# xuelunshen/gim

Hardware: AMD Instinct MI355X
Metric: image-pairs/sec at 640x480 (higher is better)
Workload: dtype fp16

## Files before the change

gim_amd/_lib.py:

```python
import ctypes
import os

_HERE = os.path.dirname(os.path.abspath(__file__))
LIB_PATH = os.path.join(_HERE, "lib", "libgimhip.so")
if os.environ.get("GIM_LIB"):
    LIB_PATH = os.environ["GIM_LIB"] if os.path.isabs(os.environ["GIM_LIB"]) else os.path.join(os.path.dirname(_HERE), os.environ["GIM_LIB"])

GIM_F32, GIM_BF16, GIM_F16 = 0, 1, 2
ACT_NONE, ACT_RELU, ACT_LEAKY, ACT_ELU1, ACT_GELU = 0, 1, 2, 3, 4

c_void_p, c_int, c_int64, c_float = ctypes.c_void_p, ctypes.c_int, ctypes.c_int64, ctypes.c_float


class ConvArgs(ctypes.Structure):
    _fields_ = [
        ("x", c_void_p), ("w", c_void_p), ("ktab", c_void_p), ("bias", c_void_p), ("res", c_void_p),
        ("y", c_void_p), ("x_bytes", c_int64),
        ("B", c_int), ("H", c_int), ("W", c_int), ("Ho", c_int), ("Wo", c_int),
        ("stride", c_int), ("pad", c_int), ("ldx", c_int), ("ldy", c_int), ("ldres", c_int),
        ("N", c_int), ("npad", c_int), ("kpad", c_int), ("act", c_int), ("act_cols", c_int), ("res_mod", c_int),
        ("dtype", c_int), ("out_dtype", c_int), ("res_dtype", c_int), ("use_lds_dma", c_int),
        ("ups", c_void_p), ("ups_h", c_int), ("ups_w", c_int), ("ups_ld", c_int),
        ("health", c_void_p),
        ("split16", c_int), ("pad_", c_int),
# ... 106 lines not shown
    "gim_resize_bilinear": (c_int, [c_void_p] * 2 + [c_int] * 10 + [c_void_p]),
    "gim_resize_image": (c_int, [c_void_p] * 2 + [c_int] * 9 + [c_void_p]),
    "gim_grid_sample": (c_int, [c_void_p] * 3 + [c_int] * 9 + [c_void_p]),
    "gim_dkm_disp_emb": (c_int, [c_void_p] * 4 + [c_int] * 6 + [c_void_p]),
    "gim_local_corr": (c_int, [c_void_p] * 4 + [c_int] * 10 + [c_void_p]),
    "gim_dwconv5x5_bn_relu": (c_int, [c_void_p] * 5 + [c_int] * 9 + [c_void_p]),
    "gim_dwconv5x5_pw": (c_int, [c_void_p] * 7 + [c_int] * 7 + [c_void_p]),
    "gim_row_norms": (c_int, [c_void_p] * 2 + [c_int] * 4 + [c_void_p]),
    "gim_cos_kernel_finish": (c_int, [c_void_p] * 3 + [c_int] * 4 + [c_float] * 3 + [c_void_p]),
    "gim_gp_solve_ws_bytes": (c_int64, [c_int] * 3),
    "gim_gp_solve": (c_int, [c_void_p] * 4 + [c_int] * 5 + [c_void_p]),
    "gim_gp_posterior_f64_ws_bytes": (c_int64, [c_int] * 4),
    "gim_gp_posterior_f64": (c_int, [c_void_p] * 5 + [c_int] * 6 + [c_float] * 3 + [c_void_p]),
    "gim_global_avgpool": (c_int, [c_void_p] * 2 + [c_int] * 7 + [c_void_p]),
    "gim_cab_scale_add": (c_int, [c_void_p] * 4 + [c_int] * 8 + [c_void_p]),
    "gim_dkm_flow_update": (c_int, [c_void_p] * 3 + [c_int64, c_int, c_float, c_float, c_int, c_int, c_void_p]),
    "gim_dkm_grid_coords": (c_int, [c_void_p] + [c_int] * 3 + [c_void_p]),
    "gim_dkm_match_post": (c_int, [c_void_p] * 10 + [c_int] * 2 + [c_void_p]),
    "gim_dkm_black_mask": (c_int, [c_void_p] * 2 + [c_int] * 4 + [c_void_p]),
    "gim_kde": (c_int, [c_void_p] * 2 + [c_int, c_float, c_void_p]),
    "gim_cls_to_flow": (c_int, [c_void_p] * 3 + [c_int] * 3 + [c_void_p]),
    "gim_dense_to_pixels": (c_int, [c_void_p] * 3 + [c_int] + [c_float] * 4 + [c_void_p]),
    "gim_weighted_sample_ws_bytes": (c_int64, [c_int]),
    "gim_weighted_sample": (c_int, [c_void_p] * 3 + [c_int, c_int, ctypes.c_uint32, c_void_p]),
    "gim_ppm_pool": (c_int, [c_void_p] * 2 + [c_int] * 6 + [c_void_p]),
    "gim_ppm_upsample_concat": (c_int, [c_void_p] * 2 + [c_int] * 7 + [c_void_p]),
    "gim_seg_head_argmax": (c_int, [c_void_p] * 4 + [c_int] * 7 + [c_void_p]),
    "gim_slot_copy": (c_int, [c_void_p] * 4 + [c_int, c_int64, c_int, c_int, c_void_p]),
    "gim_nn_match_ws_bytes": (c_int64, [c_int] * 4),
    "gim_nn_match": (c_int, [c_void_p] * 2 + [c_int] * 4 + [c_float] + [c_void_p] * 5),
    "gim_conv3x3_halo_tiles": (c_int, [ctypes.POINTER(ConvArgs), c_void_p, c_void_p, c_int, c_void_p]),
    "gim_fine_tile_list_max_flags": (c_int, []),
    "gim_fine_tile_list": (c_int, [c_void_p] * 4 + [c_int] * 7 + [c_void_p, c_void_p, c_int, c_void_p]),
    "gim_ransac_score": (c_int, [c_void_p] * 5 + [c_int, c_int, ctypes.c_double, c_void_p, c_void_p]),
    "gim_ransac_mask": (c_int, [c_void_p] * 4 + [c_int, ctypes.c_double, c_void_p, c_void_p]),
}


class GimHipError(RuntimeError):
    pass


def _load():
    if not os.path.exists(LIB_PATH):
        raise ImportError(
            f"libgimhip.so not found at {LIB_PATH}: the HIP extension is required (no CPU fallback). "
            "Build it with `python -m gim_amd.build` (needs hipcc, gfx950).")
    try:
        import torch
    except ImportError:
        pass
    lib = ctypes.CDLL(LIB_PATH)
    for name, (res, args) in PROTOTYPES.items():
        fn = getattr(lib, name)
        fn.restype = res
        fn.argtypes = args
    if lib.gim_version() != ABI_VERSION:
        raise ImportError(f"{LIB_PATH} is ABI revision {lib.gim_version()}, gim_amd/_lib.py binds revision {ABI_VERSION}: rebuild with `python -m gim_amd.build`")
    return lib


lib = _load()


def check(rc, what=""):
    if rc != 0:
# ... 3 lines not shown
```

gim_amd/csrc/emit.hip:

```cpp
#include "gim_common.h"

namespace {

struct Segs { gim_copy_segs s; };

__global__ void __launch_bounds__(256) copy_segments_kernel(const Segs a) {
    const int k = blockIdx.y;
    const char* src = (const char*)a.s.src[k];
    char* dst = (char*)a.s.dst[k];
    const int64_t n = a.s.bytes[k];
    const int64_t t = (int64_t)blockIdx.x * blockDim.x + threadIdx.x, nt = (int64_t)gridDim.x * blockDim.x;
    const bool vec = (((uintptr_t)src | (uintptr_t)dst) & 15) == 0;
    const int64_t nv = vec ? n >> 4 : 0;
    for (int64_t i = t; i < nv; i += nt) ((uint4*)dst)[i] = src ? ((const uint4*)src)[i] : make_uint4(0u, 0u, 0u, 0u);
    for (int64_t i = (nv << 4) + t; i < n; i += nt) dst[i] = src ? src[i] : (char)0;
}

__global__ void __launch_bounds__(256) pack_matches_kernel(const int64_t* __restrict__ m_bids, const float2* __restrict__ mk0,
                                                           const float2* __restrict__ mk1, const float* __restrict__ conf,
                                                           const int64_t* __restrict__ pair_ids, int64_t pid_base,
                                                           float* __restrict__ out, int M) {
    const int m = blockIdx.x * blockDim.x + threadIdx.x;
    if (m >= M) return;
    const int64_t b = m_bids[m];
    const float pid = (float)(pair_ids ? pair_ids[b] : pid_base + b);
    const float2 p0 = mk0[m], p1 = mk1[m];
    float* o = out + (size_t)m * 6;
    *(float2*)(o + 0) = make_float2(pid, p0.x);
    *(float2*)(o + 2) = make_float2(p0.y, p1.x);
    *(float2*)(o + 4) = make_float2(p1.y, conf[m]);
}

constexpr int TL_THREADS = 1024, TL_MAX_FLAGS = 32768;

__global__ void __launch_bounds__(TL_THREADS) fine_tile_list_kernel(const int64_t* __restrict__ b_ids, const int64_t* __restrict__ i_ids,
                                                                  const int64_t* __restrict__ j_ids, const int* __restrict__ count, int cap,
                                                                  int bs, int w0c, int w1c, int stride, int H, int W,
                                                                  int* __restrict__ tiles, int* __restrict__ n_tiles, int tiles_cap) {
    __shared__ unsigned char flags[TL_MAX_FLAGS];
    __shared__ int part[TL_THREADS];
    const int t = threadIdx.x;
    const int tiles_x = (W + 31) / 32, tiles_y = (H + 7) / 8, per_img = tiles_x * tiles_y, nflags = 2 * bs * per_img;
    for (int i = t; i < nflags; i += TL_THREADS) flags[i] = 0;
    __syncthreads();
    int M = count[0];
    M = M < 0 ? 0 : (M < cap ? M : cap);
    for (int m = t; m < M; m += TL_THREADS) {
        const int64_t b = b_ids[m];
        if (b < 0 || b >= bs) continue;
#pragma unroll
        for (int side = 0; side < 2; ++side) {
            const int64_t cell = side ? j_ids[m] : i_ids[m];
            const int wc = side ? w1c : w0c;
            if (cell < 0 || cell >= (int64_t)wc * ((H + stride - 1) / stride)) continue;
            const int cy = (int)cell / wc, cx = (int)cell - cy * wc;
            int y0 = cy * stride - 3, y1 = cy * stride + 3, x0 = cx * stride - 3, x1 = cx * stride + 3;
            y0 = y0 < 0 ? 0 : y0; x0 = x0 < 0 ? 0 : x0;
            y1 = y1 > H - 1 ? H - 1 : y1; x1 = x1 > W - 1 ? W - 1 : x1;
            if (y0 > y1 || x0 > x1) continue;
            const int img = side * bs + (int)b;
            for (int ty = y0 >> 3; ty <= (y1 >> 3); ++ty)
                for (int tx = x0 >> 5; tx <= (x1 >> 5); ++tx) flags[(img * tiles_y + ty) * tiles_x + tx] = 1;
        }
    }
    __syncthreads();
    const int per = (nflags + TL_THREADS - 1) / TL_THREADS;
    const int lo = t * per < nflags ? t * per : nflags, hi = lo + per < nflags ? lo + per : nflags;
    int n = 0;
    for (int i = lo; i < hi; ++i) n += flags[i];
    part[t] = n;
    __syncthreads();
    for (int d = 1; d < TL_THREADS; d <<= 1) {
        const int v = t >= d ? part[t - d] : 0;
        __syncthreads();
        part[t] += v;
        __syncthreads();
    }
    int o = part[t] - n;
    for (int i = lo; i < hi; ++i)
        if (flags[i]) {
            if (o < tiles_cap) tiles[o] = i;
            ++o;
        }
    if (t == TL_THREADS - 1) n_tiles[0] = part[t] < tiles_cap ? part[t] : tiles_cap;
}

}

extern "C" int gim_fine_tile_list_max_flags(void) { return TL_MAX_FLAGS; }

extern "C" int gim_fine_tile_list(const int64_t* b_ids, const int64_t* i_ids, const int64_t* j_ids, const int* count, int cap, int bs,
                                  int w0c, int w1c, int stride, int H, int W, int* tiles, int* n_tiles, int tiles_cap, gim_stream_t stream) {
    GIM_REQUIRE(b_ids && i_ids && j_ids && count && tiles && n_tiles, "gim_fine_tile_list: NULL pointer");
    GIM_REQUIRE(cap >= 0 && bs > 0 && w0c > 0 && w1c > 0 && stride > 0 && H > 0 && W > 0, "gim_fine_tile_list: bad geometry");
    const int64_t nflags = 2ll * bs * ((W + 31) / 32) * ((H + 7) / 8);
    GIM_REQUIRE(nflags <= TL_MAX_FLAGS, "gim_fine_tile_list: %lld patches exceed the %d flags of the one-workgroup kernel", (long long)nflags, TL_MAX_FLAGS);
    GIM_REQUIRE(tiles_cap >= nflags, "gim_fine_tile_list: the list holds %d entries, the maps have %lld patches", tiles_cap, (long long)nflags);
    hipLaunchKernelGGL(fine_tile_list_kernel, dim3(1), dim3(TL_THREADS), 0, (hipStream_t)stream, b_ids, i_ids, j_ids, count, cap, bs, w0c, w1c,
                       stride, H, W, tiles, n_tiles, tiles_cap);
    return gim_check_launch("fine_tile_list_kernel");
}

extern "C" int gim_copy_segments(const gim_copy_segs* sp, gim_stream_t stream) {
    GIM_REQUIRE(sp, "gim_copy_segments: NULL args");
    GIM_REQUIRE(sp->n >= 0 && sp->n <= GIM_MAX_COPY_SEGS, "gim_copy_segments: n=%d outside [0, %d]", sp->n, GIM_MAX_COPY_SEGS);
    int64_t mx = 0;
    for (int k = 0; k < sp->n; ++k) {
        GIM_REQUIRE(sp->bytes[k] >= 0 && (sp->bytes[k] == 0 || sp->dst[k]), "gim_copy_segments: segment %d: bad size / NULL dst", k);
        mx = sp->bytes[k] > mx ? sp->bytes[k] : mx;
    }
    if (sp->n == 0 || mx == 0) return GIM_OK;
    Segs a;
    a.s = *sp;
    int64_t blocks = (mx / 16 + 255) / 256;
    blocks = blocks < 1 ? 1 : (blocks > 1024 ? 1024 : blocks);
    hipLaunchKernelGGL(copy_segments_kernel, dim3((unsigned)blocks, (unsigned)sp->n), dim3(256), 0, (hipStream_t)stream, a);
    return gim_check_launch("copy_segments_kernel");
}

extern "C" int gim_pack_matches(const int64_t* m_bids, const float* mkpts0, const float* mkpts1, const float* mconf,
                                const int64_t* pair_ids, int64_t pid_base, float* out, int M, gim_stream_t stream) {
    GIM_REQUIRE(M >= 0, "gim_pack_matches: M=%d", M);
    if (M == 0) return GIM_OK;
    GIM_REQUIRE(m_bids && mkpts0 && mkpts1 && mconf && out, "gim_pack_matches: NULL pointer");
    hipLaunchKernelGGL(pack_matches_kernel, dim3((unsigned)((M + 255) / 256)), dim3(256), 0, (hipStream_t)stream, m_bids,
                       (const float2*)mkpts0, (const float2*)mkpts1, mconf, pair_ids, pid_base, out, M);
    return gim_check_launch("pack_matches_kernel");
}
```

gim_amd/loftr/loftr.py:

```python
import collections
import contextlib
import math
import os
import warnings

import torch
import torch.nn as nn

from .. import ops
from ..switches import flag
from .._lib import ACT_ELU1, ACT_LEAKY, ACT_NONE, ACT_RELU, GIM_F16, GimHipError
from ..packing import (PRECISION_DTYPE as _DT, PackedStem, cstore, is_half, pack_bneck, pack_bneck_ds, pack_bneck_tail, pack_conv, pack_conv_split, pack_fine_fused,
                       pack_stem7x7, pack_token_mlp, pack_token_emit, split_channels, torch_dtype)

SPLIT16_WSCALE, SPLIT16_LIMIT = 4096.0, 65504.0


def _half(v):
    return (v - 1) // 2 + 1


def split16_weight_overflow(packs):
    named = [(k, v.w) for k, v in packs.items() if hasattr(v, "w") and torch.is_tensor(v.w) and v.w.dtype == torch.float32 and v.w.numel()]
    if not named:
# ... 140 lines not shown
        if config["fine_concat_coarse_feat"]:
            raise NotImplementedError("fine_concat_coarse_feat=True is not used by gim_loftr and is not built")
        self.precision = _precision_from(config)
        self.coarse_sim = self._check_sim((config.get("coarse_sim") or flag("coarse_sim", "") or self.precision).lower())
        self.stem_fp16 = flag("stem_fp16", True, config)
        self.stem_split = flag("stem_split", "auto", config)
        self.stem_kernel = flag("stem_kernel", True, config)
        self.fp16_overflowed = False
        self.split_overflowed = False
        self.backbone = _ResNetFPN_8_2(config["resnetfpn"])
        self.loftr_coarse = _LocalFeatureTransformer(config["coarse"])
        self.loftr_fine = _LocalFeatureTransformer(config["fine"])
        self.W = config["fine_window_size"]
        self.use_lds_dma = flag("lds_dma", True, config)
        self.fine_fused = flag("fine_fused", True, config)
        self.token_fused = flag("token_fused", True, config)
        self.fine_dev_count = flag("fine_dev_count", True, config)
        self._count_pin = None
        self.token_emit = flag("token_emit", True, config)
        self.bneck_fused = flag("bneck_fused", True, config)
        self.bneck_tail = flag("bneck_tail", True, config)
        self.bneck_ds = flag("bneck_ds", True, config)
        self.bneck_tail_ds = flag("bneck_tail_ds", True, config)
        self.depth_groups = flag("depth_groups", 1, config)
        self.l3_chains = flag("l3_chains", 2, config)
        self.fp32_split = flag("fp32_split", True, config)
        self.trunk_chains = flag("trunk_chains", False, config)
        self.tf_chains = flag("tf_chains", 2, config)
        self.kv_fused = flag("kv_fused", True, config)
        self.q_local = flag("q_local", True, config)
        self.kv_init = flag("kv_init", True, config)
        self.pos_fused = flag("pos_fused", True, config)
        self.fine_sparse = flag("fine_sparse", True, config)
        self._packed = None
        self._health = None
        self._health_sync_left = 3
        self._split16 = None
        self._packed_key = None
        self._pe_cache = {}
        self.debug = None
        self.use_graph = flag("graph", True, config)
        self.graph_cache_size = max(1, flag("graph_cache", 4, config))
        self._graphs = collections.OrderedDict()
        self._seen = collections.OrderedDict()
        self._generation = 0
        self._weights_gen = getattr(self, "_weights_gen", 0)
        if config.get("weight") is not None:
            self.load_state_dict(torch.load(config["weight"], map_location="cpu"))

    def load_state_dict(self, state_dict, *args, **kwargs):
        for k in list(state_dict.keys()):
            if k.startswith("model."):
                state_dict[k.replace("model.", "", 1)] = state_dict.pop(k)
            if k.startswith("matcher."):
                state_dict[k.replace("matcher.", "", 1)] = state_dict.pop(k)
        self._invalidate()
        return super().load_state_dict(state_dict, *args, **kwargs)

    def _invalidate(self):
        self._packed = None
        self._health_sync_left = 3
        self._weights_gen = getattr(self, "_weights_gen", 0) + 1
        if hasattr(self, "_graphs"):
            self._graphs.clear()
            self._seen.clear()

# ... 153 lines not shown
            self._pe_cache[key] = pe.permute(1, 2, 0).reshape(h * w, d_model).contiguous().to(device)
        return self._pe_cache[key]

    @contextlib.contextmanager
    def _launch_scope(self, device):
        if self.precision == "fp32" and self.fp32_split and device is not None:
            self._prepack(device)
        outer = self._split16
        self._split16 = True if (self.precision == "fp32" and self.fp32_split) else None
        try:
            yield
        finally:
            self._split16 = outer

    def _conv(self, x, pk, act=ACT_NONE, **kw):
        return ops.conv2d(x, pk, act, lds_dma=self.use_lds_dma, health=self._health, split16=self._split16, **kw)

    def _linear(self, x, pk, y, act=ACT_NONE, **kw):
        ops.linear(x, pk, y, act, self.use_lds_dma, health=self._health, split16=self._split16, **kw)

    def _to_nhwc(self, images, dt, out=None):
        H, W = images[0].shape[2:]
        B = sum(im.shape[0] for im in images)
        split = self._split()
        if out is None:
            cs = 8 if self._stem_k() else cstore(split_channels(images[0].shape[1]) if split else 3, dt)
            out = torch.empty(B, H, W, cs, dtype=torch_dtype(dt), device=images[0].device)
        off = 0
        for im in images:
            (ops.nchw_to_nhwc_split if split else ops.nchw_to_nhwc)(im, out, off)
            off += im.shape[0]
        return out

    def _backbone(self, P, x, dt, fine_tail=True):
        x1, x2, x3_out = self._backbone_trunk(P, x, dt)
        x1_out = self._fpn_fine(P, x1, x2, x3_out)
        return x3_out, (self._fpn_fine_tail(P, x1_out) if fine_tail else x1_out)

    def _backbone_trunk(self, P, x, dt):
        B = x.shape[0]
        K = self.l3_chains if (self.debug is None and self.l3_chains > 1 and B % self.l3_chains == 0) else 1
        if K > 1:
            h4, w4 = _half(_half(x.shape[1])), _half(_half(x.shape[2]))
            if (B // K * h4 * w4) % 256 != 0 or (B // K * _half(h4) * _half(w4)) % 256 != 0:
                K = 1
        whole = K > 1 and self.trunk_chains
        G = K if whole else (self.depth_groups if (self.debug is None and self.depth_groups > 1 and B % self.depth_groups == 0) else 1)
        o3 = None
        if G > 1:
            n = B // G
            H1, W1 = _half(x.shape[1]), _half(x.shape[2])
            H2, W2 = _half(H1), _half(W1)
            tdt = torch_dtype(dt)
            x1 = torch.empty(B, H1, W1, P["l1.2.c3"].n_store, dtype=tdt, device=x.device)
            x2 = torch.empty(B, H2, W2, P["l2.3.c3"].n_store, dtype=tdt, device=x.device)
            if self.bneck_tail and "l2.3.tail" in P and (n * H2 * W2) % 256 == 0 and n * H2 * W2 * 1024 < (1 << 32) - 16:
                o3 = torch.empty(B, H2, W2, P["l3.0.c1"].n_store, dtype=tdt, device=x.device)

        def trunk12_group(g):
            sl = slice(g * n, (g + 1) * n)
            a1, a2, ao = self._trunk12(P, x[sl], dt, out=(x1[sl], x2[sl], o3[sl] if o3 is not None else None))
            assert (ao is None) == (o3 is None)
            for dst, src in ((x1, a1), (x2, a2), (o3, ao)):
                if src is not None and src.data_ptr() != dst[sl].data_ptr():
                    ops.copy_segments([(src.contiguous(), dst[sl])])

        if G == 1:
            x1, x2, o3 = self._trunk12(P, x, dt)
# ... 53 lines not shown
            p = f"l{li}.{bi}."
            last = bi == nblk - 1
            outs = out_last if last else None
            if o is None:
                o = self._conv(x, P[p + "c1"], ACT_RELU)
            if fuse and self.bneck_ds and (p + "fused_ds") in P and x.shape[3] == 64 and x.is_contiguous():
                x, o = ops.bneck64_ds(o, x, P[p + "fused_ds"], out=outs, health=self._health)
                continue
            rows_ds = x.shape[0] * _half(x.shape[1]) * _half(x.shape[2])
            if (self.bneck_tail and self.bneck_tail_ds and (p + "tail_ds") in P and x.is_contiguous() and x.shape[3] == 256
                    and rows_ds % 256 == 0 and rows_ds * 512 * 2 < (1 << 32) - 16):
                o = self._conv(o, P[p + "c2"], ACT_RELU)
                x, o = ops.bneck_tail_ds(o, x, P[p + "tail_ds"], out=outs, health=self._health)
                continue
            idn = self._conv(x, P[p + "ds"], ACT_NONE) if (p + "ds") in P else x
            if fuse:
                x, o = ops.bneck64(o, idn, P[p + "fused"], True, out=outs, health=self._health)
                continue
            o = self._conv(o, P[p + "c2"], ACT_RELU)
            rows = o.shape[0] * o.shape[1] * o.shape[2]
            if self.bneck_tail and (p + "tail") in P and rows % 256 == 0 and rows * 4 * o.shape[3] * 2 < (1 << 32) - 16:
                if li == 3 and last:
                    x, x3_out = ops.bneck_tail(o, idn.contiguous(), P[p + "tail"], ACT_NONE, store_x=self.debug is not None, out=outs,
                                               health=self._health)
                    o = None
                else:
                    x, o = ops.bneck_tail(o, idn.contiguous(), P[p + "tail"], out=outs, health=self._health)
                continue
            x = self._conv(o, P[p + "c3"], ACT_RELU, res=idn)
            o = None
        return x, o, x3_out

    def _fpn_fine(self, P, x1, x2, x3_out):
        x2_out = self._conv(x2, P["l2o"], ups=x3_out)
        x2_out = self._conv(self._conv(x2_out, P["l2o2a"], ACT_LEAKY), P["l2o2b"])
        return self._conv(x1, P["l1o"], ups=x2_out)

    def _fine_halo(self, P, h2, w2):
        return bool(self.fine_sparse and is_half(self._dt()) and self.use_lds_dma and ops.HALO and P["l1o2a"].halo is not None
                    and P["l1o2b"].halo is not None and h2 % 8 == 0 and w2 % 32 == 0)

    def _fpn_fine_tail(self, P, x1_out, tiles=None, n_tiles=None):
        B, H, W, _ = x1_out.shape
        if self._fine_halo(P, H, W):
            mid = torch.empty(B, H, W, P["l1o2a"].n_store, dtype=x1_out.dtype, device=x1_out.device)
            f = torch.empty(B, H, W, P["l1o2b"].n_store, dtype=x1_out.dtype, device=x1_out.device)
            ops.conv3x3_halo(x1_out, P["l1o2a"], mid, ACT_LEAKY, tiles=tiles, n_tiles=n_tiles)
            ops.conv3x3_halo(mid, P["l1o2b"], f, ACT_NONE, tiles=tiles, n_tiles=n_tiles)
            return f
        assert tiles is None
        return self._conv(self._conv(x1_out, P["l1o2a"], ACT_LEAKY), P["l1o2b"])

    def _fine_sparse_ok(self, P, xs):
        if self.debug is not None or len(xs) != 1:
            return False
        B, H, W = xs[0].shape[:3]
        h2, w2 = _half(H), _half(W)
        h8, w8 = _half(_half(h2)), _half(_half(w2))
        return self._fine_halo(P, h2, w2) and h2 == 4 * h8 and w2 == 4 * w8 and B * (h2 // 8) * (w2 // 32) <= ops.FINE_TILE_MAX_FLAGS

    def _fine_tail_sparse(self, P, x1_out, cr, bs):
        _, H, W, _ = x1_out.shape
        tiles, n_tiles = ops.fine_tile_list(cr.b_ids, cr.i_ids, cr.j_ids, cr.count, bs, cr.args.w0c, cr.args.w1c, 4, H, W)
        return self._fpn_fine_tail(P, x1_out, tiles, n_tiles)

    class _TfBuffers:
        _LAZY = {"QKV": 3, "QKV2": 3, "MSG": 1, "MRG": 1, "HID": 2, "MLP": 1}

        def __init__(self, R, C, tdt, dev):
            f32 = torch.float32
            self._shape = (R, C, tdt, dev)
            self.X32 = torch.empty(R, C, dtype=f32, device=dev)
            self.CAT = torch.empty(R, 2 * C, dtype=tdt, device=dev)
            self.ws = None
            self.MASK = None
            self.pos = None
            self.pos_all = None

        def __getattr__(self, name):
            w = type(self)._LAZY.get(name)
            if w is None:
                raise AttributeError(name)
            R, C, tdt, dev = self._shape
            t = torch.empty(R, w * C, dtype=tdt, device=dev)
            setattr(self, name, t)
            return t

    def _encoder_layer(self, P, p, T, xs, ss, nb, L, S, H, have_q=False, with_q_of_source=False):
        C = T.X32.shape[1]
        x_t, s_t = T.CAT[xs, :C], T.CAT[ss, :C]
        if xs == ss:
            self._linear(x_t, P[p + "qkv"], T.QKV[xs], ACT_ELU1, act_cols=2 * C)
        else:
            if not have_q:
                self._linear(x_t, P[p + "q_proj"], T.QKV[xs, :C], ACT_ELU1)
            if with_q_of_source:
                self._linear(s_t, P[p + "qkv"], T.QKV[ss], ACT_ELU1, act_cols=2 * C)
# ... 212 lines not shown
            if T.pos[sd] is not None:
                feat, pe = T.pos[sd]
                ops.posenc_add(feat, pe, T.X32[rows[sd]], T.CAT[rows[sd], :C])
                T.pos[sd] = None

    def _transformer(self, P, name, tf, T, n0, L, n1, S):
        r0, r1 = slice(0, n0 * L), slice(n0 * L, n0 * L + n1 * S)
        rall = slice(0, n0 * L + n1 * S)
        H = tf.nhead
        if (self.token_emit and self.token_fused and (name + ".emit", L == S) in P and L % 64 == 0 and S % 64 == 0 and H == 8
                and T.X32.shape[1] == 256 and all(f"{name}{li}.tok" in P for li in range(len(tf.layer_names)))):
            return self._transformer_emit(P, name, tf, T, n0, L, n1, S)
        self._posenc(T, (r0, r1))
        for li, kind in enumerate(tf.layer_names):
            p = f"{name}{li}."
            if kind == "self":
                if L == S:
                    self._encoder_layer(P, p, T, rall, rall, n0 + n1, L, S, H)
                else:
                    self._encoder_layer(P, p, T, r0, r0, n0, L, L, H)
                    self._encoder_layer(P, p, T, r1, r1, n1, S, S, H)
            else:
                self._encoder_layer(P, p, T, r0, r1, n0, L, S, H, with_q_of_source=True)
                self._encoder_layer(P, p, T, r1, r0, n1, S, L, H, have_q=True)

    def _coarse_stage(self, xs, bs, scale0, scale1, mask0=None, mask1=None, count=None):
        dev = xs[0].device
        if count is None:
            count = torch.zeros(2 + bs, dtype=torch.int32, device=dev)
        self._health = self._health_word(count[1:2])
        P = self._prepack(dev)
        if len(xs) == 1:
            if self._fine_sparse_ok(P, xs):
                c_all, x1_out = self._extract_stage(P, xs[0], fine_tail=False)
                st = self._match_stage(P, c_all[:bs], c_all[bs:], None, None, c_all, bs, xs[0].shape[1], scale0, scale1, mask0, mask1, count)
                f_all = self._fine_tail_sparse(P, x1_out, st["cr"], bs)
                st["f0"], st["f1"] = f_all[:bs], f_all[bs:]
                return st
            c_all, f_all = self._extract_stage(P, xs[0])
            c0, c1 = c_all[:bs], c_all[bs:]
            f0, f1 = f_all[:bs], f_all[bs:]
        else:
            c_all = None
            c0, f0 = self._extract_stage(P, xs[0])
            c1, f1 = self._extract_stage(P, xs[1])
        return self._match_stage(P, c0, c1, f0, f1, c_all, bs, xs[0].shape[1], scale0, scale1, mask0, mask1, count)

    def _health_word(self, word):
        split = ops.FP32_SPLIT if self._split16 is None else self._split16
        return word if (self.precision == "fp16" or (self.precision == "fp32" and split)) else None

    def _extract_stage(self, P, x, fine_tail=True):
        return self._backbone(P, x, self._dt(), fine_tail)

    def _match_stage(self, P, c0, c1, f0, f1, c_all, bs, H0, scale0, scale1, mask0, mask1, count):
        dev = c0.device
        dt = self._dt()
        self._health = self._health_word(count[1:2])
        tdt = torch_dtype(dt)
        cfg = self.config
        hw0_c, hw1_c = c0.shape[1:3], c1.shape[1:3]
        C = cfg["coarse"]["d_model"]
        L, S = hw0_c[0] * hw0_c[1], hw1_c[0] * hw1_c[1]
        T = self._TfBuffers(bs * (L + S), C, tdt, dev)
        r0, r1 = slice(0, bs * L), slice(bs * L, bs * (L + S))
        if mask0 is not None:
            T.MASK = torch.empty(bs * (L + S), dtype=torch.uint8, device=dev)
            T.MASK[r0].copy_(mask0.reshape(-1))
            T.MASK[r1].copy_(mask1.reshape(-1))
        T.pos = [(c0.reshape(-1, C), self._pos_encoding(C, *hw0_c, dev)), (c1.reshape(-1, C), self._pos_encoding(C, *hw1_c, dev))]
        T.pos_all = c_all.reshape(-1, C) if c_all is not None else None
        self._transformer(P, "c", self.loftr_coarse, T, bs, L, bs, S)
        mc = cfg["match_coarse"]
        scale = H0 / hw0_c[0]
        if is_half(dt) and self.coarse_sim == self.precision:
            fc0 = T.CAT[r0].view(bs, L, 2 * C)[:, :, :C]
            fc1 = T.CAT[r1].view(bs, S, 2 * C)[:, :, :C]
        else:
            fc0, fc1 = T.X32[r0].view(bs, L, C), T.X32[r1].view(bs, S, C)
        cr = ops.coarse_match(fc0, fc1, hw0_c, hw1_c, scale,
                              mc["dsmax_temperature"], mc["thr"], mc["border_rm"], scale0, scale1,
                              T.MASK[r0] if mask0 is not None else None, T.MASK[r1] if mask0 is not None else None, count=count)
        self._health = None
        return {"c0": c0, "c1": c1, "f0": f0, "f1": f1, "cr": cr,
                "feat_c0": T.X32[r0].view(bs, L, C), "feat_c1": T.X32[r1].view(bs, S, C)}

    def _graph_key(self, color0, color1, scale0, mask0):
        return (tuple(color0.shape), tuple(color1.shape), scale0 is not None, mask0 is not None, self.precision, bool(self.fp32_split),
                bool(self.fine_sparse), self.coarse_sim, self._img_dt(), self._split(), self._stem_k(), str(color0.device))

    def _stage_graphed(self, key, fill, warm, stage, bs, dev, scale0, scale1, mask0, mask1):
        ent = self._graphs.get(key)
        if ent is None:
            warm()
            sin = [fill(None),
                   scale0.clone().float() if scale0 is not None else None,
                   scale1.clone().float() if scale1 is not None else None,
                   mask0.clone() if mask0 is not None else None, mask1.clone() if mask1 is not None else None,
                   torch.zeros(2 + bs, dtype=torch.int32, device=dev)]
            torch.cuda.synchronize()
            graph = torch.cuda.CUDAGraph()
            with torch.cuda.graph(graph, capture_error_mode="thread_local"):
                out = stage(*sin)
            while len(self._graphs) >= self.graph_cache_size:
                self._graphs.popitem(last=False)
            ent = self._graphs[key] = (graph, sin, out)
        else:
            self._graphs.move_to_end(key)
            fill(ent[1][0])
        graph, sin, out = ent
        small = []
        if scale0 is not None:
            small += [(scale0, sin[1]), (scale1, sin[2])]
        if mask0 is not None:
            small += [(mask0, sin[3]), (mask1, sin[4])]
        ops.copy_segments(small)
        graph.replay()
        return out

    def _run_stage(self, key, graphed, eager):
        counted = self.use_graph and self.debug is None
        if counted and (key in self._graphs or self._seen.get(key, 0) >= 1):
# ... 30 lines not shown

    @torch.no_grad()
    def forward(self, data):
        c0 = data.get("color0")
        with self._launch_scope(c0.device if torch.is_tensor(c0) and c0.is_cuda else None):
            return self._forward(data)

    def _forward(self, data):
        for k in ("image0", "image1", "color0", "color1"):
            if k not in data:
                raise KeyError(f"LoFTR.forward needs data[{k!r}] (loftr.py:54-63)")
        color0, color1 = data["color0"], data["color1"]
        if not color0.is_cuda:
            raise GimHipError("gim_amd LoFTR runs on the HIP device only (no CPU fallback): move the inputs "
                              "and the module to 'cuda'")
        dev = color0.device
        self._prepack(dev)
        color0 = color0.contiguous().float()
        color1 = color1.contiguous().float()
        scale0, scale1, mask0, mask1 = self._pair_inputs(data, dev, (color0.shape[0], color0.shape[2] // 8, color0.shape[3] // 8),
                                                         (color1.shape[0], color1.shape[2] // 8, color1.shape[3] // 8))
        data.update({"bs": data["image0"].size(0),
                     "hw0_i": data["image0"].shape[2:], "hw1_i": data["image1"].shape[2:]})
        bs = data["bs"]
        groups = [[color0, color1]] if color0.shape[2:] == color1.shape[2:] else [[color0], [color1]]

        def to_nhwc(out):
            if out is None:
                return [self._to_nhwc(g, self._img_dt()) for g in groups]
            for g, x in zip(groups, out):
                self._to_nhwc(g, self._img_dt(), out=x)

        def warm():
            self._prepack(dev)
            for c in (color0, color1):
                self._pos_encoding(self.config["coarse"]["d_model"], _half(_half(_half(c.shape[2]))), _half(_half(_half(c.shape[3]))), dev)

        key = self._graph_key(color0, color1, scale0, mask0)
        st, graphed = self._run_stage(
            key, lambda: self._stage_graphed(key, to_nhwc, warm, lambda xs, *rest: self._coarse_stage(xs, color0.shape[0], *rest), color0.shape[0], dev,
                                             scale0, scale1, mask0, mask1),
            lambda: self._coarse_stage(to_nhwc(None), bs, scale0, scale1, mask0, mask1))
        return self._finish(data, st, graphed, scale1, lambda: self.forward(data))

    def _finish(self, data, st, graphed, scale1, rerun):
        dev = st["c0"].device
        c0, c1, f0, f1, cr = st["c0"], st["c1"], st["f0"], st["f1"], st["cr"]
        if self.debug is not None:
            self.debug.update({k: st[k] for k in ("c0", "c1", "f0", "f1", "feat_c0", "feat_c1")})
        hw0_c, hw1_c = c0.shape[1:3], c1.shape[1:3]
        hw0_f, hw1_f = f0.shape[1:3], f1.shape[1:3]
        data.update({"hw0_c": torch.Size(hw0_c), "hw1_c": torch.Size(hw1_c),
                     "hw0_f": torch.Size(hw0_f), "hw1_f": torch.Size(hw1_f)})

        fine = None
        dev_count = (self.fine_dev_count and self.fine_fused and self.debug is None and "fine_fused" in self._prepack(dev)
                     and f0.dtype in ops.HALF)
        if self._count_pin is None:
            self._count_pin = torch.empty(2, dtype=torch.int32).pin_memory()
        if dev_count:
            self._count_pin.copy_(cr.count[:2], non_blocking=True)
            ev = torch.cuda.Event()
            ev.record()
            cap = cr.b_ids.numel()
            fine = self._fine_level(f0, f1, cr.b_ids, cr.i_ids, cr.j_ids, cr.mkpts1_c, scale1, "scale0" in data,
                                    hw0_c, hw1_c, data["hw0_i"], True, count=cr.count)
            ev.synchronize()
# ... 202 lines not shown
```

gim_amd/ops.py:

```python
import ctypes
import os

import torch

from . import _lib
from ._lib import ACT_ELU1, ACT_GELU, ACT_LEAKY, ACT_NONE, ACT_RELU, GIM_BF16, GIM_F16, GIM_F32, check, lib
from .packing import elem_size, torch_dtype
from .switches import flag

_DT = {torch.float32: GIM_F32, torch.bfloat16: GIM_BF16, torch.float16: GIM_F16}
HALF = (torch.bfloat16, torch.float16)


PROFILE = None
PROFILE_FUSED = None


def _stream():
    return ctypes.c_void_p(torch.cuda.current_stream().cuda_stream)


class _Timed:

    def __init__(self, family, flops):
# ... 261 lines not shown
        launch = lambda: check(lib.gim_conv3x3_halo_tiles(ctypes.byref(a), _p(tiles), _p(n_tiles), tiles.numel(), _stream()),
                               "gim_conv3x3_halo_tiles")
    if PROFILE is None:
        launch()
        return
    e0, e1 = torch.cuda.Event(enable_timing=True), torch.cuda.Event(enable_timing=True)
    e0.record()
    launch()
    e1.record()
    label = f"{pk.cin}->{pk.cout} k3s1 M={B * H * W} halo"
    if tiles is None:
        PROFILE.append((e0, e1, 2.0 * B * H * W * pk.cout * pk.cin * 9, label))
    else:
        PROFILE.append((e0, e1, 2.0 * int(n_tiles[0].item()) * 256 * pk.cout * pk.cin * 9, label + " sparse"))


FINE_TILE_MAX_FLAGS = lib.gim_fine_tile_list_max_flags()


def fine_tile_list(b_ids, i_ids, j_ids, count, bs, w0c, w1c, stride, H, W, tiles=None, n_tiles=None):
    _req_cuda(b_ids, i_ids, j_ids, count, tiles, n_tiles)
    assert b_ids.dtype == i_ids.dtype == j_ids.dtype == torch.int64 and count.dtype == torch.int32
    assert b_ids.is_contiguous() and i_ids.is_contiguous() and j_ids.is_contiguous()
    cap = min(b_ids.numel(), i_ids.numel(), j_ids.numel())
    total = 2 * bs * ((H + 7) // 8) * ((W + 31) // 32)
    if tiles is None:
        tiles = torch.empty(total, dtype=torch.int32, device=b_ids.device)
    if n_tiles is None:
        n_tiles = torch.empty(1, dtype=torch.int32, device=b_ids.device)
    assert tiles.dtype == n_tiles.dtype == torch.int32 and tiles.is_contiguous()
    check(lib.gim_fine_tile_list(_p(b_ids), _p(i_ids), _p(j_ids), _p(count), cap, bs, w0c, w1c, stride, H, W, _p(tiles), _p(n_tiles),
                                 tiles.numel(), _stream()), "gim_fine_tile_list")
    return tiles, n_tiles


def linear(x, pk, y, act=ACT_NONE, lds_dma=True, act_cols=0, health=None, split16=None):
    rows = x.shape[0]
    conv_rows(x, pk, (1, 1, rows, 1, rows), y, act, None, 0, lds_dma, act_cols, health=health, split16=split16)


def upsample2x_add(x, y):
    _req_cuda(x, y)
    B, h, w, C = x.shape
    assert y.shape == (B, 2 * h, 2 * w, C) and x.dtype == y.dtype
    check(lib.gim_upsample2x_add(_p(x), _p(y), B, h, w, C, C, C, gim_dtype(x), _stream()), "gim_upsample2x_add")


def posenc_add(x, pe, out_f32, out_t):
    _req_cuda(x, pe, out_f32, out_t)
    R, C = x.shape
    check(lib.gim_posenc_add(_p(x), _p(pe), _p(out_f32), _p(out_t), R, pe.shape[0], C, x.stride(0),
                             out_f32.stride(0) if out_f32 is not None else 4,
                             out_t.stride(0) if out_t is not None else 4, gim_dtype(x), _stream()), "gim_posenc_add")


def layernorm_residual(x, gamma, beta, res, out_f32, out_t, eps=1e-5):
    _req_cuda(x, gamma, beta, res, out_f32, out_t)
    R, C = x.shape
    dt = gim_dtype(out_t) if out_t is not None else GIM_F32
    check(lib.gim_layernorm_residual(_p(x), _p(gamma), _p(beta), _p(res), _p(out_f32), _p(out_t), R, C,
                                     x.stride(0), res.stride(0) if res is not None else 4,
                                     out_f32.stride(0) if out_f32 is not None else 4,
                                     out_t.stride(0) if out_t is not None else 4, gim_dtype(x), dt, eps, _stream()),
          "gim_layernorm_residual")


# ... 789 lines not shown
```

include/gim_hip.h:

```cpp
#ifndef GIM_HIP_H
#define GIM_HIP_H
#include <stdint.h>

#ifdef __cplusplus
extern "C" {
#endif

typedef void* gim_stream_t;

enum { GIM_F32 = 0, GIM_BF16 = 1, GIM_F16 = 2 };
enum { GIM_ACT_NONE = 0, GIM_ACT_RELU = 1, GIM_ACT_LEAKY = 2, GIM_ACT_ELU1 = 3 , GIM_ACT_GELU = 4  };
enum { GIM_OK = 0, GIM_ERR_INVALID = -1, GIM_ERR_LAUNCH = -2, GIM_ERR_UNSUPPORTED = -3 };

int gim_version(void);
const char* gim_last_error(void);
int gim_ktile_bytes(void);
int gim_npad_granule(void);

int gim_nchw_to_nhwc(const float* src, void* dst, int B, int C, int H, int W, int cpad, int ld,
                     int b_off, int dtype, gim_stream_t stream);
int gim_nchw_to_nhwc_split(const float* src, void* dst, int B, int C, int H, int W, int ld, int b_off, int dtype,
                           gim_stream_t stream);

int64_t gim_stem7x7_weight_bytes(int split);
// ... 224 lines not shown
    const float* match_b;
    void* ws;
    int64_t* matches0;
    int64_t* matches1;
    float* mscores0;
    float* mscores1;
    int32_t* pos;
    int32_t* count;
    int B, M, N, C;
    int ld_desc;
    float threshold;
} gim_lg_assign_args;
int64_t gim_lg_assign_ws_bytes(int B, int M, int N, int C);
int gim_lg_assign(const gim_lg_assign_args* a, gim_stream_t stream);
int gim_lg_log_assignment(const gim_lg_assign_args* a, float* out, gim_stream_t stream);
int gim_lg_emit_matches(const int64_t* matches0, const float* mscores0, const int32_t* pos,
                        const int32_t* count, const float* kpts0, const float* kpts1, const float* scale0,
                        const float* scale1, int64_t* matches, float* scores, float* mkpts0, float* mkpts1,
                        int64_t* m_bids, int B, int M, int N, gim_stream_t stream);

enum { GIM_MAX_COPY_SEGS = 12 };
typedef struct gim_copy_segs {
    const void* src[12];
    void* dst[12];
    int64_t bytes[12];
    int n;
} gim_copy_segs;
int gim_copy_segments(const gim_copy_segs* segs, gim_stream_t stream);
int gim_pack_matches(const int64_t* m_bids, const float* mkpts0, const float* mkpts1, const float* mconf,
                     const int64_t* pair_ids, int64_t pid_base, float* out, int M, gim_stream_t stream);
int gim_fine_tile_list_max_flags(void);
int gim_fine_tile_list(const int64_t* b_ids, const int64_t* i_ids, const int64_t* j_ids, const int* count, int cap, int bs,
                       int w0c, int w1c, int stride, int H, int W, int* tiles, int* n_tiles, int tiles_cap, gim_stream_t stream);


int gim_maxpool3x3s2(const void* x, void* y, int B, int H, int W, int C, int ldx, int ldy, int dtype,
                     gim_stream_t stream);
int gim_resize_bilinear(const void* x, void* y, int B, int h, int w, int Ho, int Wo, int C, int ldx, int ldy,
                        int dtype, int out_dtype, gim_stream_t stream);
int gim_resize_image(const float* x, void* y, int B, int C, int h, int w, int Ho, int Wo, int cpad, int b_off,
                     int out_dtype, gim_stream_t stream);
int gim_grid_sample(const void* feat, const float* grid_xy, void* out, int B, int h, int w, int Ho, int Wo, int C,
                    int ldf, int ldo, int dtype, gim_stream_t stream);
int gim_dkm_disp_emb(const float* flow, const float* wgt, const float* bias, void* out, int B, int h, int w, int E,
                     int ldo, int out_dtype, gim_stream_t stream);
int gim_local_corr(const void* f0, const void* f1, const float* flow, void* out, int B, int h, int w, int C, int r,
                   int ld0, int ld1, int ldo, int dtype, int out_dtype, gim_stream_t stream);
int gim_dwconv5x5_bn_relu(const void* x, const float* wgt, const float* scale, const float* shift, void* y, int B,
                          int H, int W, int Cin, int Cout, int cpad, int ldx, int ldy, int dtype, gim_stream_t stream);
int gim_dwconv5x5_pw(const void* x, const float* wgt, const float* scale, const float* shift, const void* pw_w, const float* pw_b, void* y,
                     int B, int H, int W, int cs, int ldx, int ldy, int dtype, gim_stream_t stream);
int gim_row_norms(const void* x, float* out, int rows, int C, int ld, int dtype, gim_stream_t stream);
int gim_cos_kernel_finish(float* k, const float* nx, const float* ny, int B, int n, int m, int ld, float T, float eps,
                          float diag_add, gim_stream_t stream);
int64_t gim_gp_solve_ws_bytes(int B, int n, int nrhs);
int gim_gp_solve(const float* K, const float* F, float* Xt, void* ws, int B, int n, int ldk, int nrhs, int npad,
                 gim_stream_t stream);
int64_t gim_gp_posterior_f64_ws_bytes(int B, int n, int d, int nrhs);
int gim_gp_posterior_f64(const float* X, const float* Y, const float* F, float* mu, void* ws, int B, int n, int d, int ldx,
                         int nrhs, int ld_mu, float T, float eps, float sigma, gim_stream_t stream);
int gim_global_avgpool(const void* x, float* out, int B, int HW, int C, int ld, int ldo, int c_off, int dtype,
                       gim_stream_t stream);
int gim_cab_scale_add(const float* g, const void* x1, const void* x2, void* out, int B, int HW, int C, int ldg, int ld1,
                      int ld2, int ldo, int dtype, gim_stream_t stream);
int gim_dkm_flow_update(float* flow, float* cert, const void* d, int64_t npix, int ldd, float sx, float sy,
                        int cert_init, int dtype, gim_stream_t stream);
// ... 38 lines not shown
```

Baseline: 917.8.

## Compute FPN quarter-resolution tail only on tiles feeding matched fine windows

Extends the sparse fine-stage approach to the 1/4-resolution FPN refinement convs (l2o2a/l2o2b). After coarse matching, a single kernel builds two tile lists, one for 1/2 resolution and one for the dilated 1/4-resolution footprint, and the quarter-res 3x3 convs run through the halo-tile path over only those tiles. The goal is to skip convolution work in regions no fine window reads. In exchange, the backbone is split around coarse matching, persistent zeroed buffers are kept per shape and per graph, and the kernel adds more bookkeeping. Correctness relies on the dilated footprint math covering the bilinear upsample support.

```diff
diff --git a/gim_amd/_lib.py b/gim_amd/_lib.py
--- a/gim_amd/_lib.py
+++ b/gim_amd/_lib.py
@@ -162,6 +162,7 @@
     "gim_conv3x3_halo_tiles": (c_int, [ctypes.POINTER(ConvArgs), c_void_p, c_void_p, c_int, c_void_p]),
     "gim_fine_tile_list_max_flags": (c_int, []),
     "gim_fine_tile_list": (c_int, [c_void_p] * 4 + [c_int] * 7 + [c_void_p, c_void_p, c_int, c_void_p]),
+    "gim_fine_tile_lists": (c_int, [c_void_p] * 4 + [c_int] * 9 + [c_void_p, c_void_p, c_int] * 2 + [c_void_p]),
     "gim_ransac_score": (c_int, [c_void_p] * 5 + [c_int, c_int, ctypes.c_double, c_void_p, c_void_p]),
     "gim_ransac_mask": (c_int, [c_void_p] * 4 + [c_int, ctypes.c_double, c_void_p, c_void_p]),
 }
diff --git a/gim_amd/csrc/emit.hip b/gim_amd/csrc/emit.hip
--- a/gim_amd/csrc/emit.hip
+++ b/gim_amd/csrc/emit.hip
@@ -33,6 +33,38 @@
 
 constexpr int TL_THREADS = 1024, TL_MAX_FLAGS = 32768;
 
+__device__ __forceinline__ void tl_mark(unsigned char* flags, int img, int tiles_y, int tiles_x, int y0, int y1, int x0, int x1) {
+    for (int ty = y0 >> 3; ty <= (y1 >> 3); ++ty)
+        for (int tx = x0 >> 5; tx <= (x1 >> 5); ++tx) flags[(img * tiles_y + ty) * tiles_x + tx] = 1;
+}
+
+__device__ __forceinline__ void tl_compact(const unsigned char* flags, int nflags, int* part, int* __restrict__ tiles, int* __restrict__ n_tiles,
+                                           int tiles_cap) {
+    const int t = threadIdx.x;
+    const int per = (nflags + TL_THREADS - 1) / TL_THREADS;
+    const int lo = t * per < nflags ? t * per : nflags, hi = lo + per < nflags ? lo + per : nflags;
+    int n = 0;
+    for (int i = lo; i < hi; ++i) n += flags[i];
+    part[t] = n;
+    __syncthreads();
+    for (int d = 1; d < TL_THREADS; d <<= 1) {
+        const int v = t >= d ? part[t - d] : 0;
+        __syncthreads();
+        part[t] += v;
+        __syncthreads();
+    }
+    int o = part[t] - n;
+    for (int i = lo; i < hi; ++i)
+        if (flags[i]) {
+            if (o < tiles_cap) tiles[o] = i;
+            ++o;
+        }
+    if (t == TL_THREADS - 1) n_tiles[0] = part[t] < tiles_cap ? part[t] : tiles_cap;
+    __syncthreads();
+}
+
+__device__ __forceinline__ int tl_clamp(int v, int lo, int hi) { return v < lo ? lo : (v > hi ? hi : v); }
+
 __global__ void __launch_bounds__(TL_THREADS) fine_tile_list_kernel(const int64_t* __restrict__ b_ids, const int64_t* __restrict__ i_ids,
                                                                   const int64_t* __restrict__ j_ids, const int* __restrict__ count, int cap,
                                                                   int bs, int w0c, int w1c, int stride, int H, int W,
@@ -58,31 +90,52 @@
             y0 = y0 < 0 ? 0 : y0; x0 = x0 < 0 ? 0 : x0;
             y1 = y1 > H - 1 ? H - 1 : y1; x1 = x1 > W - 1 ? W - 1 : x1;
             if (y0 > y1 || x0 > x1) continue;
-            const int img = side * bs + (int)b;
-            for (int ty = y0 >> 3; ty <= (y1 >> 3); ++ty)
-                for (int tx = x0 >> 5; tx <= (x1 >> 5); ++tx) flags[(img * tiles_y + ty) * tiles_x + tx] = 1;
+            tl_mark(flags, side * bs + (int)b, tiles_y, tiles_x, y0, y1, x0, x1);
         }
     }
     __syncthreads();
-    const int per = (nflags + TL_THREADS - 1) / TL_THREADS;
-    const int lo = t * per < nflags ? t * per : nflags, hi = lo + per < nflags ? lo + per : nflags;
-    int n = 0;
-    for (int i = lo; i < hi; ++i) n += flags[i];
-    part[t] = n;
+    tl_compact(flags, nflags, part, tiles, n_tiles, tiles_cap);
+}
+
+__global__ void __launch_bounds__(TL_THREADS) fine_tile_lists_kernel(const int64_t* __restrict__ b_ids, const int64_t* __restrict__ i_ids,
+                                                                   const int64_t* __restrict__ j_ids, const int* __restrict__ count, int cap,
+                                                                   int bs, int w0c, int w1c, int stride, int H, int W, int HB, int WB,
+                                                                   int* __restrict__ tiles_a, int* __restrict__ n_tiles_a, int cap_a,
+                                                                   int* __restrict__ tiles_b, int* __restrict__ n_tiles_b, int cap_b) {
+    __shared__ unsigned char flags[TL_MAX_FLAGS];
+    __shared__ int part[TL_THREADS];
+    const int t = threadIdx.x;
+    const int ax = (W + 31) / 32, ay = (H + 7) / 8, nflags_a = 2 * bs * ax * ay;
+    const int bx = (WB + 31) / 32, by = (HB + 7) / 8, nflags_b = 2 * bs * bx * by;
+    unsigned char* const flags_b = flags + nflags_a;
+    for (int i = t; i < nflags_a + nflags_b; i += TL_THREADS) flags[i] = 0;
     __syncthreads();
-    for (int d = 1; d < TL_THREADS; d <<= 1) {
-        const int v = t >= d ? part[t - d] : 0;
-        __syncthreads();
-        part[t] += v;
-        __syncthreads();
+    int M = count[0];
+    M = M < 0 ? 0 : (M < cap ? M : cap);
+    for (int m = t; m < M; m += TL_THREADS) {
+        const int64_t b = b_ids[m];
+        if (b < 0 || b >= bs) continue;
+#pragma unroll
+        for (int side = 0; side < 2; ++side) {
+            const int64_t cell = side ? j_ids[m] : i_ids[m];
+            const int wc = side ? w1c : w0c;
+            if (cell < 0 || cell >= (int64_t)wc * ((H + stride - 1) / stride)) continue;
+            const int cy = (int)cell / wc, cx = (int)cell - cy * wc;
+            const int img = side * bs + (int)b;
+            if (cy * stride - 3 <= H - 1 && cx * stride - 3 <= W - 1)
+                tl_mark(flags, img, ay, ax, tl_clamp(cy * stride - 3, 0, H - 1), tl_clamp(cy * stride + 3, 0, H - 1),
+                        tl_clamp(cx * stride - 3, 0, W - 1), tl_clamp(cx * stride + 3, 0, W - 1));
+            if (cy * stride - 4 > H - 1 || cx * stride - 4 > W - 1) continue;
+            const int y_lo = tl_clamp(cy * stride - 4, 0, H - 1), y_hi = tl_clamp(cy * stride + 4, 0, H - 1);
+            const int x_lo = tl_clamp(cx * stride - 4, 0, W - 1), x_hi = tl_clamp(cx * stride + 4, 0, W - 1);
+            const int r0 = y_lo * (HB - 1) / (H - 1) - 1, r1 = y_hi * (HB - 1) / (H - 1) + 2;
+            const int c0 = x_lo * (WB - 1) / (W - 1) - 1, c1 = x_hi * (WB - 1) / (W - 1) + 2;
+            tl_mark(flags_b, img, by, bx, tl_clamp(r0, 0, HB - 1), tl_clamp(r1, 0, HB - 1), tl_clamp(c0, 0, WB - 1), tl_clamp(c1, 0, WB - 1));
+        }
     }
-    int o = part[t] - n;
-    for (int i = lo; i < hi; ++i)
-        if (flags[i]) {
-            if (o < tiles_cap) tiles[o] = i;
-            ++o;
-        }
-    if (t == TL_THREADS - 1) n_tiles[0] = part[t] < tiles_cap ? part[t] : tiles_cap;
+    __syncthreads();
+    tl_compact(flags, nflags_a, part, tiles_a, n_tiles_a, cap_a);
+    tl_compact(flags_b, nflags_b, part, tiles_b, n_tiles_b, cap_b);
 }
 
 }
@@ -99,6 +152,21 @@
     hipLaunchKernelGGL(fine_tile_list_kernel, dim3(1), dim3(TL_THREADS), 0, (hipStream_t)stream, b_ids, i_ids, j_ids, count, cap, bs, w0c, w1c,
                        stride, H, W, tiles, n_tiles, tiles_cap);
     return gim_check_launch("fine_tile_list_kernel");
+}
+
+extern "C" int gim_fine_tile_lists(const int64_t* b_ids, const int64_t* i_ids, const int64_t* j_ids, const int* count, int cap, int bs,
+                                   int w0c, int w1c, int stride, int H, int W, int HB, int WB, int* tiles_a, int* n_tiles_a, int cap_a,
+                                   int* tiles_b, int* n_tiles_b, int cap_b, gim_stream_t stream) {
+    GIM_REQUIRE(b_ids && i_ids && j_ids && count && tiles_a && n_tiles_a && tiles_b && n_tiles_b, "gim_fine_tile_lists: NULL pointer");
+    GIM_REQUIRE(cap >= 0 && bs > 0 && w0c > 0 && w1c > 0 && stride > 0 && HB > 0 && WB > 0, "gim_fine_tile_lists: bad geometry");
+    GIM_REQUIRE(H == 2 * HB && W == 2 * WB, "gim_fine_tile_lists: the second level must be half the first (%d x %d against %d x %d)", HB, WB, H, W);
+    const int64_t na = 2ll * bs * ((W + 31) / 32) * ((H + 7) / 8), nb = 2ll * bs * ((WB + 31) / 32) * ((HB + 7) / 8);
+    GIM_REQUIRE(na + nb <= TL_MAX_FLAGS, "gim_fine_tile_lists: %lld patches exceed the %d flags of the one-workgroup kernel", (long long)(na + nb), TL_MAX_FLAGS);
+    GIM_REQUIRE(cap_a >= na && cap_b >= nb, "gim_fine_tile_lists: the lists hold %d / %d entries, the maps have %lld / %lld patches", cap_a, cap_b,
+                (long long)na, (long long)nb);
+    hipLaunchKernelGGL(fine_tile_lists_kernel, dim3(1), dim3(TL_THREADS), 0, (hipStream_t)stream, b_ids, i_ids, j_ids, count, cap, bs, w0c, w1c,
+                       stride, H, W, HB, WB, tiles_a, n_tiles_a, cap_a, tiles_b, n_tiles_b, cap_b);
+    return gim_check_launch("fine_tile_lists_kernel");
 }
 
 extern "C" int gim_copy_segments(const gim_copy_segs* sp, gim_stream_t stream) {
diff --git a/gim_amd/loftr/loftr.py b/gim_amd/loftr/loftr.py
--- a/gim_amd/loftr/loftr.py
+++ b/gim_amd/loftr/loftr.py
@@ -196,6 +196,9 @@
         self.kv_init = flag("kv_init", True, config)
         self.pos_fused = flag("pos_fused", True, config)
         self.fine_sparse = flag("fine_sparse", True, config)
+        self.fpn_sparse = flag("fpn_sparse", True, config)
+        self._fpn_eager = None
+        self._fpn_fresh = None
         self._packed = None
         self._health = None
         self._health_sync_left = 3
@@ -415,8 +418,11 @@
             off += im.shape[0]
         return out
 
-    def _backbone(self, P, x, dt, fine_tail=True):
+    def _backbone(self, P, x, dt, fine_tail=True, fpn_tail=True):
         x1, x2, x3_out = self._backbone_trunk(P, x, dt)
+        if not fpn_tail:
+            assert not fine_tail
+            return x3_out, (x1, self._fpn_lateral2(P, x2, x3_out))
         x1_out = self._fpn_fine(P, x1, x2, x3_out)
         return x3_out, (self._fpn_fine_tail(P, x1_out) if fine_tail else x1_out)
 
@@ -536,9 +542,25 @@
         return x, o, x3_out
 
     def _fpn_fine(self, P, x1, x2, x3_out):
-        x2_out = self._conv(x2, P["l2o"], ups=x3_out)
-        x2_out = self._conv(self._conv(x2_out, P["l2o2a"], ACT_LEAKY), P["l2o2b"])
+        x2_out = self._fpn_quarter_tail(P, self._fpn_lateral2(P, x2, x3_out))
         return self._conv(x1, P["l1o"], ups=x2_out)
+
+    def _fpn_lateral2(self, P, x2, x3_out):
+        return self._conv(x2, P["l2o"], ups=x3_out)
+
+    def _fpn_halo(self, P, h4, w4):
+        return bool(self.fpn_sparse and self.fine_sparse and is_half(self._dt()) and self.use_lds_dma and ops.HALO and P["l2o2a"].halo is not None
+                    and P["l2o2b"].halo is not None and h4 % 8 == 0 and w4 % 32 == 0)
+
+    def _fpn_quarter_tail(self, P, x2_lat, tiles=None, n_tiles=None, out=None):
+        B, H, W, _ = x2_lat.shape
+        if self._fpn_halo(P, H, W):
+            mid, y = out if out is not None else (torch.empty(B, H, W, P[k].n_store, dtype=x2_lat.dtype, device=x2_lat.device) for k in ("l2o2a", "l2o2b"))
+            ops.conv3x3_halo(x2_lat, P["l2o2a"], mid, ACT_LEAKY, tiles=tiles, n_tiles=n_tiles)
+            ops.conv3x3_halo(mid, P["l2o2b"], y, ACT_NONE, tiles=tiles, n_tiles=n_tiles)
+            return y
+        assert tiles is None
+        return self._conv(self._conv(x2_lat, P["l2o2a"], ACT_LEAKY), P["l2o2b"])
 
     def _fine_halo(self, P, h2, w2):
         return bool(self.fine_sparse and is_half(self._dt()) and self.use_lds_dma and ops.HALO and P["l1o2a"].halo is not None
@@ -567,6 +589,44 @@
         _, H, W, _ = x1_out.shape
         tiles, n_tiles = ops.fine_tile_list(cr.b_ids, cr.i_ids, cr.j_ids, cr.count, bs, cr.args.w0c, cr.args.w1c, 4, H, W)
         return self._fpn_fine_tail(P, x1_out, tiles, n_tiles)
+
+    def _fpn_sparse_ok(self, P, xs):
+        if not self._fine_sparse_ok(P, xs):
+            return False
+        B, H, W = xs[0].shape[:3]
+        h2, w2 = _half(H), _half(W)
+        h4, w4 = _half(h2), _half(w2)
+        return (self._fpn_halo(P, h4, w4) and h2 == 2 * h4 and w2 == 2 * w4
+                and B * ((h2 // 8) * (w2 // 32) + (h4 // 8) * (w4 // 32)) <= ops.FINE_TILE_MAX_FLAGS)
+
+    def _fpn_buffers(self, P, B, h4, w4, tdt, dev, warm_graph=False):
+        key = (B, h4, w4, P["l2o2a"].n_store, P["l2o2b"].n_store, tdt, str(dev))
+
+        def zeros():
+            return tuple(torch.zeros(B, h4, w4, n, dtype=tdt, device=dev) for n in key[3:5])
+
+        if warm_graph:
+            self._fpn_eager = self._fpn_fresh = None
+            self._fpn_fresh = (key, zeros())
+            return None
+        if torch.cuda.is_current_stream_capturing():
+            fresh, self._fpn_fresh = self._fpn_fresh, None
+            assert fresh is not None and fresh[0] == key, "the graph's warm-up made no buffers for this shape"
+            return fresh[1]
+        self._fpn_fresh = None
+        if self._fpn_eager is None or self._fpn_eager[0] != key:
+            self._fpn_eager = None
+            self._fpn_eager = (key, zeros())
+        return self._fpn_eager[1]
+
+    def _fpn_tail_sparse(self, P, head, cr, bs):
+        x1, x2_lat = head
+        B, h4, w4, _ = x2_lat.shape
+        (t2, n2), (t4, n4) = ops.fine_tile_lists(cr.b_ids, cr.i_ids, cr.j_ids, cr.count, bs, cr.args.w0c, cr.args.w1c, 4, 2 * h4, 2 * w4)
+        out = self._fpn_buffers(P, B, h4, w4, x2_lat.dtype, x2_lat.device)
+        x2_out = self._fpn_quarter_tail(P, x2_lat, t4, n4, out=out)
+        x1_out = self._conv(x1, P["l1o"], ups=x2_out)
+        return self._fpn_fine_tail(P, x1_out, t2, n2), out
 
     class _TfBuffers:
         _LAZY = {"QKV": 3, "QKV2": 3, "MSG": 1, "MRG": 1, "HID": 2, "MLP": 1}
@@ -845,9 +905,13 @@
         P = self._prepack(dev)
         if len(xs) == 1:
             if self._fine_sparse_ok(P, xs):
-                c_all, x1_out = self._extract_stage(P, xs[0], fine_tail=False)
+                fpn = self._fpn_sparse_ok(P, xs)
+                c_all, head = self._extract_stage(P, xs[0], fine_tail=False, fpn_tail=not fpn)
                 st = self._match_stage(P, c_all[:bs], c_all[bs:], None, None, c_all, bs, xs[0].shape[1], scale0, scale1, mask0, mask1, count)
-                f_all = self._fine_tail_sparse(P, x1_out, st["cr"], bs)
+                if fpn:
+                    f_all, st["fpn_buffers"] = self._fpn_tail_sparse(P, head, st["cr"], bs)
+                else:
+                    f_all = self._fine_tail_sparse(P, head, st["cr"], bs)
                 st["f0"], st["f1"] = f_all[:bs], f_all[bs:]
                 return st
             c_all, f_all = self._extract_stage(P, xs[0])
@@ -863,8 +927,8 @@
         split = ops.FP32_SPLIT if self._split16 is None else self._split16
         return word if (self.precision == "fp16" or (self.precision == "fp32" and split)) else None
 
-    def _extract_stage(self, P, x, fine_tail=True):
-        return self._backbone(P, x, self._dt(), fine_tail)
+    def _extract_stage(self, P, x, fine_tail=True, fpn_tail=True):
+        return self._backbone(P, x, self._dt(), fine_tail, fpn_tail)
 
     def _match_stage(self, P, c0, c1, f0, f1, c_all, bs, H0, scale0, scale1, mask0, mask1, count):
         dev = c0.device
@@ -900,7 +964,7 @@
 
     def _graph_key(self, color0, color1, scale0, mask0):
         return (tuple(color0.shape), tuple(color1.shape), scale0 is not None, mask0 is not None, self.precision, bool(self.fp32_split),
-                bool(self.fine_sparse), self.coarse_sim, self._img_dt(), self._split(), self._stem_k(), str(color0.device))
+                bool(self.fine_sparse), bool(self.fpn_sparse), self.coarse_sim, self._img_dt(), self._split(), self._stem_k(), str(color0.device))
 
     def _stage_graphed(self, key, fill, warm, stage, bs, dev, scale0, scale1, mask0, mask1):
         ent = self._graphs.get(key)
@@ -997,7 +1061,11 @@
                 self._to_nhwc(g, self._img_dt(), out=x)
 
         def warm():
-            self._prepack(dev)
+            P = self._prepack(dev)
+            if len(groups) == 1:
+                B, (H, W) = 2 * color0.shape[0], color0.shape[2:]
+                if self._fpn_sparse_ok(P, [torch.empty(B, H, W, 1, device="meta")]):
+                    self._fpn_buffers(P, B, _half(_half(H)), _half(_half(W)), torch_dtype(self._dt()), dev, warm_graph=True)
             for c in (color0, color1):
                 self._pos_encoding(self.config["coarse"]["d_model"], _half(_half(_half(c.shape[2]))), _half(_half(_half(c.shape[3]))), dev)
 
diff --git a/gim_amd/ops.py b/gim_amd/ops.py
--- a/gim_amd/ops.py
+++ b/gim_amd/ops.py
@@ -317,6 +317,21 @@
     check(lib.gim_fine_tile_list(_p(b_ids), _p(i_ids), _p(j_ids), _p(count), cap, bs, w0c, w1c, stride, H, W, _p(tiles), _p(n_tiles),
                                  tiles.numel(), _stream()), "gim_fine_tile_list")
     return tiles, n_tiles
+
+
+def fine_tile_lists(b_ids, i_ids, j_ids, count, bs, w0c, w1c, stride, H, W):
+    _req_cuda(b_ids, i_ids, j_ids, count)
+    assert b_ids.dtype == i_ids.dtype == j_ids.dtype == torch.int64 and count.dtype == torch.int32
+    assert b_ids.is_contiguous() and i_ids.is_contiguous() and j_ids.is_contiguous()
+    assert H % 2 == 0 and W % 2 == 0
+    cap = min(b_ids.numel(), i_ids.numel(), j_ids.numel())
+    HB, WB = H // 2, W // 2
+    ta = torch.empty(2 * bs * ((H + 7) // 8) * ((W + 31) // 32), dtype=torch.int32, device=b_ids.device)
+    tb = torch.empty(2 * bs * ((HB + 7) // 8) * ((WB + 31) // 32), dtype=torch.int32, device=b_ids.device)
+    n = torch.empty(2, dtype=torch.int32, device=b_ids.device)
+    check(lib.gim_fine_tile_lists(_p(b_ids), _p(i_ids), _p(j_ids), _p(count), cap, bs, w0c, w1c, stride, H, W, HB, WB, _p(ta), _p(n[0:1]),
+                                  ta.numel(), _p(tb), _p(n[1:2]), tb.numel(), _stream()), "gim_fine_tile_lists")
+    return (ta, n[0:1]), (tb, n[1:2])
 
 
 def linear(x, pk, y, act=ACT_NONE, lds_dma=True, act_cols=0, health=None, split16=None):
diff --git a/include/gim_hip.h b/include/gim_hip.h
--- a/include/gim_hip.h
+++ b/include/gim_hip.h
@@ -280,6 +280,9 @@
 int gim_fine_tile_list_max_flags(void);
 int gim_fine_tile_list(const int64_t* b_ids, const int64_t* i_ids, const int64_t* j_ids, const int* count, int cap, int bs,
                        int w0c, int w1c, int stride, int H, int W, int* tiles, int* n_tiles, int tiles_cap, gim_stream_t stream);
+int gim_fine_tile_lists(const int64_t* b_ids, const int64_t* i_ids, const int64_t* j_ids, const int* count, int cap, int bs,
+                        int w0c, int w1c, int stride, int H, int W, int HB, int WB, int* tiles_a, int* n_tiles_a, int cap_a,
+                        int* tiles_b, int* n_tiles_b, int cap_b, gim_stream_t stream);
 
 
 int gim_maxpool3x3s2(const void* x, void* y, int B, int H, int W, int C, int ldx, int ldy, int dtype,
```

Result: no change. 922.4, median of 6 (+0.5%).
